# ucla-mobility/QuantV2X

Measured on AMD Instinct MI355X. Metric: frames/sec/node (N-agent int8 BEV fusion), higher is better.
Workload: dtype i8

## Files before the change

quantv2x_amd/csrc/codebook_encode_cand.hip:

```cpp
#include "common.h"

namespace qv2x {
namespace {

struct CandArgs {
    const int8_t* in; const int8_t* gpack; const double* bias; const int* tables;
    uint8_t* codes; unsigned* list; unsigned* counters;
    float tau[3][3];
    int n, h, w, hw, M, levels, kc, ke, zx, gbytes, tbytes;
    float delta;
};

constexpr int NPF = 8;
constexpr int LIMBS = 3;
template <int V> struct IC { static constexpr int value = V; };

__device__ __forceinline__ double shfl_xor_f64(double v, int m) {
    const long long b = __builtin_bit_cast(long long, v);
    const int lo = __shfl_xor((int)b, m), hi = __shfl_xor((int)(b >> 32), m);
    return __builtin_bit_cast(double, ((long long)hi << 32) | (unsigned)lo);
}

template <int CT, int SEGS, int PACK>
__global__ __launch_bounds__(256) __attribute__((amdgpu_waves_per_eu(1, 1))) void encode_candidates_kernel(const CandArgs a) {
    const int lane = threadIdx.x & 63, wave = __builtin_amdgcn_readfirstlane(threadIdx.x >> 6), j = lane & 31, hf = lane >> 5;
    const int m0 = ((int)blockIdx.x * 4 + wave) * (32 * CT);

    v4i xb[CT][8];
    int m[CT];
    float n0[CT], n1[CT];
#pragma unroll
    for (int ct = 0; ct < CT; ++ct) {
        m[ct] = m0 + 32 * ct + j;
        const int mc = m[ct] < a.M ? m[ct] : a.M - 1;
        const int img = mc / a.hw, rem = mc - img * a.hw, y = rem / a.w, x = rem - y * a.w;
        const int8_t* px = a.in + ((size_t)(img * (a.h + 2) + y + 1) * (a.w + 2) + x + 1) * 256 + 16 * hf;
#pragma unroll
        for (int s = 0; s < 8; ++s) xb[ct][s] = *(const v4i*)(px + 32 * s);
        unsigned s1 = 0, s2 = 0, sad = 0;
        const unsigned zx4 = (unsigned)a.zx * 0x01010101u;
#pragma unroll
        for (int s = 0; s < 8; ++s)
#pragma unroll
            for (int d = 0; d < 4; ++d) {
                const unsigned u = (unsigned)xb[ct][s][d] ^ 0x80808080u;
                s1 = __builtin_amdgcn_udot4(u, 0x01010101u, s1, false);
                s2 = __builtin_amdgcn_udot4(u, u, s2, false);
                sad = __builtin_amdgcn_sad_u8(u, zx4, sad);
            }
        s1 += __shfl_xor(s1, 32); s2 += __shfl_xor(s2, 32); sad += __shfl_xor(sad, 32);
        const int n2 = (int)s2 - 2 * a.zx * (int)s1 + 256 * a.zx * a.zx;
        n0[ct] = a.delta * sqrtf((float)n2);
        n1[ct] = (float)sad;
    }

    const __amdgpu_buffer_rsrc_t grs = __builtin_amdgcn_make_buffer_rsrc((void*)a.gpack, 0, a.gbytes, 0x00020000);
    int wo = 0;
    const int loff = lane * 16;
    auto gload = [&](int f) __attribute__((always_inline)) { return (v4i)__builtin_amdgcn_raw_buffer_load_b128(grs, loff, wo + f * 1024, 0); };
    v4i ring[NPF];
#pragma unroll
    for (int i = 0; i < NPF; ++i) ring[i] = gload(i);

    const __amdgpu_buffer_rsrc_t brs = __builtin_amdgcn_make_buffer_rsrc((void*)a.bias, 0, a.levels * a.ke * 8, 0x00020000);
    const __amdgpu_buffer_rsrc_t trs = __builtin_amdgcn_make_buffer_rsrc((void*)a.tables, 0, a.tbytes, 0x00020000);
    int o[2][SEGS][CT] = {};
    int first[CT];
#pragma unroll
    for (int ct = 0; ct < CT; ++ct) first[ct] = 3;
    const int ntile = a.kc >> 5;
    const int tsz = a.ke * a.ke;
    auto level = [&](auto lc) __attribute__((always_inline)) {
        constexpr int l = decltype(lc)::value;
        bool weak_l[CT];
#pragma unroll
        for (int ct = 0; ct < CT; ++ct) weak_l[ct] = false;
        auto segment = [&](auto sc) __attribute__((always_inline)) {
        constexpr int sg = decltype(sc)::value;
        double best[CT], second[CT];
#pragma unroll
        for (int ct = 0; ct < CT; ++ct) best[ct] = second[ct] = 1.0e300;
        v4i qb[2][2], qt[2][l > 0 ? l * SEGS : 1][CT];
        auto issue = [&](int T, int g, int slot) __attribute__((always_inline)) {
            const int col = sg * a.kc + 32 * T + 8 * g;
            const int kofs = l * a.ke + col;
            qb[slot][0] = (v4i)__builtin_amdgcn_raw_buffer_load_b128(brs, 32 * hf, kofs * 8, 0);
            qb[slot][1] = (v4i)__builtin_amdgcn_raw_buffer_load_b128(brs, 32 * hf + 16, kofs * 8, 0);
#pragma unroll
            for (int ct = 0; ct < CT; ++ct) {
#pragma unroll
                for (int jj = 0; jj < l; ++jj)
#pragma unroll
                    for (int sp = 0; sp < SEGS; ++sp)
                        qt[slot][jj * SEGS + sp][ct] = (v4i)__builtin_amdgcn_raw_buffer_load_b128(trs, o[jj][sp][ct], ((l * (l - 1) / 2 + jj) * tsz + col) * 4, 0);
            }
        };
#pragma unroll 1
        for (int T = 0; T < ntile; ++T) {
            v16i acc[LIMBS][CT];
#pragma unroll
            for (int lb = 0; lb < LIMBS; ++lb)
#pragma unroll
                for (int ct = 0; ct < CT; ++ct)
#pragma unroll
                    for (int r = 0; r < 16; ++r) acc[lb][ct][r] = 0;
#pragma unroll
            for (int f = 0; f < LIMBS * 8; ++f) {
                const v4i A = ring[f % NPF];
#pragma unroll
                for (int ct = 0; ct < CT; ++ct) acc[f >> 3][ct] = __builtin_amdgcn_mfma_i32_32x32x32_i8(A, xb[ct][f & 7], acc[f >> 3][ct], 0, 0, 0);
                ring[f % NPF] = gload(f + NPF);
                if (f == LIMBS * 8 - 6) issue(T, 0, 0);
                __builtin_amdgcn_sched_barrier(0);
            }
            wo += LIMBS * 8 * 1024;
#pragma unroll
            for (int g = 0; g < 4; ++g) {
                if (g < 3) issue(T, g + 1, (g + 1) & 1);
                __builtin_amdgcn_sched_barrier(0);
                const int sl = g & 1;
                double b[4];
                b[0] = __builtin_bit_cast(double, ((unsigned long long)(unsigned)qb[sl][0][1] << 32) | (unsigned)qb[sl][0][0]);
                b[1] = __builtin_bit_cast(double, ((unsigned long long)(unsigned)qb[sl][0][3] << 32) | (unsigned)qb[sl][0][2]);
                b[2] = __builtin_bit_cast(double, ((unsigned long long)(unsigned)qb[sl][1][1] << 32) | (unsigned)qb[sl][1][0]);
                b[3] = __builtin_bit_cast(double, ((unsigned long long)(unsigned)qb[sl][1][3] << 32) | (unsigned)qb[sl][1][2]);
#pragma unroll
                for (int ct = 0; ct < CT; ++ct) {
#pragma unroll
                    for (int e = 0; e < 4; ++e) {
                        const int r = 4 * g + e;
                        int lo = (acc[1][ct][r] << 8) + acc[0][ct][r];
#pragma unroll
                        for (int q = 0; q < l * SEGS; ++q) lo += qt[sl][q][ct][e];
                        double c = __builtin_fma((double)lo, (double)PACK, b[e]);
                        c = __builtin_fma((double)acc[2][ct][r], 65536.0 * PACK, c);
                        second[ct] = fmin(second[ct], fmax(best[ct], c));
                        best[ct] = fmin(best[ct], c);
                    }
                }
                __builtin_amdgcn_sched_barrier(0);
            }
        }
#pragma unroll
        for (int ct = 0; ct < CT; ++ct) {
            const double ob = shfl_xor_f64(best[ct], 32), os = shfl_xor_f64(second[ct], 32);
            const double nb = fmin(best[ct], ob), ns = fmin(fmax(best[ct], ob), fmin(second[ct], os));
            const int c = (int)((long long)nb & (PACK - 1));
            if (l < 2) o[l < 2 ? l : 0][sg][ct] = ((sg * a.kc + c) * a.ke + 4 * hf) * 4;
            const float t = ((a.tau[l][0] + a.tau[l][1] * n0[ct]) + (a.tau[l][2] * n0[ct]) * n0[ct]) + n1[ct];
            weak_l[ct] |= !(ns - nb > (double)PACK * (double)ceilf(t) + (double)(PACK - 1));
            if (hf == 0 && m[ct] < a.M) a.codes[(size_t)(l * SEGS + sg) * a.M + m[ct]] = (uint8_t)c;
        }
        };
        segment(IC<0>{});
        if constexpr (SEGS > 1) segment(IC<1>{});
#pragma unroll
        for (int ct = 0; ct < CT; ++ct)
            if (weak_l[ct] && first[ct] == 3) first[ct] = l;
    };
    level(IC<0>{});
    if (a.levels > 1) level(IC<1>{});
    if (a.levels > 2) level(IC<2>{});
    unsigned long long mask[3][CT];
    unsigned cnt[3] = {0, 0, 0};
#pragma unroll
    for (int c = 0; c < 3; ++c)
#pragma unroll
        for (int ct = 0; ct < CT; ++ct) {
            mask[c][ct] = __builtin_amdgcn_ballot_w64(first[ct] == c && hf == 0 && m[ct] < a.M);
            cnt[c] += (unsigned)__builtin_popcountll(mask[c][ct]);
        }
    __shared__ unsigned wcnt[4][3], wbase[3];
    if (lane == 0) { wcnt[wave][0] = cnt[0]; wcnt[wave][1] = cnt[1]; wcnt[wave][2] = cnt[2]; }
    __syncthreads();
    if (threadIdx.x < 3) {
        const unsigned tot = wcnt[0][threadIdx.x] + wcnt[1][threadIdx.x] + wcnt[2][threadIdx.x] + wcnt[3][threadIdx.x];
        wbase[threadIdx.x] = tot ? atomicAdd(a.counters + 1 + threadIdx.x, tot) : 0u;
        if (tot) atomicAdd(a.counters, tot);
    }
    __syncthreads();
    unsigned base[3];
#pragma unroll
    for (int c = 0; c < 3; ++c) {
        base[c] = wbase[c];
        for (int w2 = 0; w2 < wave; ++w2) base[c] += wcnt[w2][c];
    }
#pragma unroll
    for (int c = 0; c < 3; ++c) {
        unsigned at = __builtin_amdgcn_readfirstlane(base[c]);
#pragma unroll
        for (int ct = 0; ct < CT; ++ct) {
            if (first[ct] == c && hf == 0 && m[ct] < a.M)
                a.list[(size_t)c * a.M + at + (unsigned)__builtin_popcountll(mask[c][ct] & ((1ull << lane) - 1ull))] = (unsigned)m[ct];
            at += (unsigned)__builtin_popcountll(mask[c][ct]);
        }
    }
}

__global__ void zero_counters_kernel(unsigned* c) { if (threadIdx.x < 4) c[threadIdx.x] = 0; }

template <int CT, int SEGS, int PACK>
void launch(const CandArgs& a, hipStream_t st) {
    encode_candidates_kernel<CT, SEGS, PACK><<<(a.M + 128 * CT - 1) / (128 * CT), 256, 0, st>>>(a);
}

template <int PACK, int MAX_SEGS>
int candidates(const char* me, const qv2x_encode_desc* d, const int8_t* in, const int8_t* g_limbs, const double* bias_packed, const int32_t* tables,
               const float* tau, uint8_t* codes, uint32_t* list, uint32_t* counters, void* stream) {
    if (!d || !in || !g_limbs || !bias_packed || !tau || !codes || !list || !counters) return fail(QV2X_EINVAL, "%s: null pointer", me);
    if (d->n <= 0 || d->h <= 0 || d->w <= 0 || d->levels < 1 || d->levels > 3) return fail(QV2X_EINVAL, "%s: 1..3 levels", me);
    const int segs = d->segs ? d->segs : 1;
    if (segs < 1 || segs > MAX_SEGS) return fail(QV2X_EINVAL, "%s: seg_num 1 .. %d (got %d; the exact entry takes seg_num 1 | 2 | 4)", me, MAX_SEGS, d->segs);
    if (d->kc < 32 || d->kc > PACK || d->kc % 32 || (segs > 1 && d->kc % 64))
        return fail(QV2X_EINVAL, "%s: dict_size a multiple of 32 up to %d (of 64 with two segments; got %d x %d)", me, PACK, segs, d->kc);
    if (d->levels > 1 && !tables) return fail(QV2X_EINVAL, "%s: the residual levels need their tables", me);
    if (d->in_zx < 0 || d->in_zx > 255) return fail(QV2X_EINVAL, "%s: in_zx outside 0..255", me);
    if (((uintptr_t)in & 15) || ((uintptr_t)g_limbs & 15) || ((uintptr_t)tables & 15) || ((uintptr_t)bias_packed & 7))
        return fail(QV2X_EALIGN, "%s: 16-byte aligned maps, limbs and tables", me);
    CandArgs a;
    a.in = in; a.gpack = g_limbs; a.bias = bias_packed; a.tables = tables; a.codes = codes; a.list = list; a.counters = counters;
    for (int l = 0; l < 3; ++l)
        for (int i = 0; i < 3; ++i) a.tau[l][i] = l < d->levels ? tau[l * 3 + i] : 0.0f;
    a.n = d->n; a.h = d->h; a.w = d->w; a.hw = d->h * d->w; a.M = d->n * a.hw; a.levels = d->levels; a.kc = d->kc; a.ke = segs * d->kc; a.zx = d->in_zx;
    a.gbytes = d->levels * (a.ke / 32) * LIMBS * 8 * 1024;
    a.tbytes = (d->levels > 1 ? d->levels * (d->levels - 1) / 2 : 1) * a.ke * a.ke * 4;
    a.delta = d->in_delta;
    hipStream_t st = (hipStream_t)stream;
    zero_counters_kernel<<<1, 64, 0, st>>>(counters);
    int dev = 0, cus = 256, v = 0;
    if (hipGetDevice(&dev) == hipSuccess && hipDeviceGetAttribute(&v, hipDeviceAttributeMultiprocessorCount, dev) == hipSuccess && v > 0) cus = v;
    const bool large = a.M >= 4 * cus * 32 * (segs == 2 ? 3 : 4) * 2;
    if (segs == 1) large ? launch<4, 1, PACK>(a, st) : launch<2, 1, PACK>(a, st);
    else if constexpr (MAX_SEGS > 1) large ? launch<3, 2, PACK>(a, st) : launch<2, 2, PACK>(a, st);
    return hip_check(hipGetLastError(), me);
}

}
}

extern "C" int qv2x_codebook_encode_candidates_i8(const qv2x_encode_desc* d, const int8_t* in, const int8_t* g_limbs, const double* bias_packed,
                                                  const int32_t* tables, const float* tau, uint8_t* codes, uint32_t* list, uint32_t* counters,
                                                  void* stream) {
    return qv2x::candidates<128, 1>("qv2x_codebook_encode_candidates_i8", d, in, g_limbs, bias_packed, tables, tau, codes, list, counters, stream);
}

extern "C" int qv2x_codebook_encode_candidates_seg_i8(const qv2x_encode_desc* d, const int8_t* in, const int8_t* g_limbs, const double* bias_packed,
                                                      const int32_t* tables, const float* tau, uint8_t* codes, uint32_t* list, uint32_t* counters,
                                                      void* stream) {
    return qv2x::candidates<256, 2>("qv2x_codebook_encode_candidates_seg_i8", d, in, g_limbs, bias_packed, tables, tau, codes, list, counters, stream);
}
```

quantv2x_amd/csrc/codebook_encode_wave.hip:

```cpp
#include "codebook_encode.h"

namespace qv2x {

namespace {

constexpr int D = ENC_D;
constexpr int RS = 260;
constexpr int NPF = 4;

__device__ __forceinline__ v16f mfma(float a, float b, v16f c) { return __builtin_amdgcn_mfma_f32_32x32x2f32(a, b, c, 0, 0, 0); }


__device__ __forceinline__ void tile_to_lds(float* __restrict__ row, int h, int T, const v16f& acc) {
#pragma unroll
    for (int rq = 0; rq < 4; ++rq) {
        float* g = row + (4 * T + rq) * 8 + 2 * h;
        *(float2*)g = make_float2(acc[4 * rq], acc[4 * rq + 2]);
        *(float2*)(g + 4) = make_float2(acc[4 * rq + 1], acc[4 * rq + 3]);
    }
}

__device__ __forceinline__ void lds_to_operand(const float* __restrict__ row, int h, float (&m)[128]) {
#pragma unroll
    for (int g = 0; g < 32; ++g) {
        const v4f v = *(const v4f*)(row + g * 8 + 4 * h);
        m[4 * g] = v.x; m[4 * g + 1] = v.y; m[4 * g + 2] = v.z; m[4 * g + 3] = v.w;
    }
}

__device__ __forceinline__ void tile_vec(const float* __restrict__ p, int h, int T, v4f (&o)[4]) {
#pragma unroll
    for (int rq = 0; rq < 4; ++rq) o[rq] = *(const v4f*)(p + 32 * T + 8 * rq + 4 * h);
}

#ifdef QV2X_ENCW_FINE
__device__ long long g_encw_fine[4096][32];
#define WFINE(k) do { if (threadIdx.x == 0 && blockIdx.x < 4096) g_encw_fine[blockIdx.x][8 * l + (k)] = __builtin_readcyclecounter(); } while (0)
#define WFINE2(k) do { if (fine2 && threadIdx.x == 0 && blockIdx.x < 4096) g_encw_fine[blockIdx.x][24 + (k)] = __builtin_readcyclecounter(); } while (0)
#define WFINE2_ARM(v) fine2 = (v)
#else
#define WFINE(k) do { } while (0)
#define WFINE2(k) do { } while (0)
#define WFINE2_ARM(v) do { } while (0)
#endif

}

template <int V> struct IC { static constexpr int value = V; };

template <bool F32IN, int SEGS, bool LIST = false>
__global__ __attribute__((amdgpu_flat_work_group_size(64, 64), amdgpu_waves_per_eu(1, 1))) void codebook_encode_wave_kernel(const EncArgs a) {
    __shared__ __attribute__((aligned(16))) float smem[32 * RS];
    const int lane = threadIdx.x, j = lane & 31, h = lane >> 5;
    float* const row = smem + j * RS;
    ListPlan plan{};
    if (LIST) plan = list_plan(a);
#pragma unroll 1
    for (int round = 0; LIST ? round * (int)gridDim.x < plan.full : round == 0; ++round) {
    const int tile = LIST ? round * (int)gridDim.x + ((round & 1) ? (int)gridDim.x - 1 - (int)blockIdx.x : (int)blockIdx.x) : (int)blockIdx.x;
    if (LIST && tile >= plan.full) continue;
    int mrow;
    bool owned;
    int start = 0;
    if (LIST) {
        int cls, i0;
        list_tile(plan, tile, cls, i0);
        owned = i0 + j < plan.n[cls];
        mrow = (int)a.list[(size_t)cls * a.M + (owned ? i0 + j : plan.n[cls] - 1)];
        start = cls;
    } else {
        mrow = a.m_lo + tile * 32 + j;
        owned = mrow < a.m_hi;
    }

    float xq[128], z[128];
    {
        int m = mrow;
        m = m < a.M ? m : a.M - 1;
        const int img = m / (a.h * a.w), rem = m - img * (a.h * a.w);
        const int y = rem / a.w, x = rem - y * a.w;
        const size_t pixel = (size_t)(img * (a.h + 2) + y + 1) * (a.w + 2) + x + 1;
        if (F32IN) {
            const v4f* sf = (const v4f*)(a.in_f32 + pixel * D);
#pragma unroll
            for (int q = 0; q < 64; ++q) {
                const v4f v = sf[q];
                xq[2 * q] = h ? v.y : v.x;
                xq[2 * q + 1] = h ? v.w : v.z;
            }
        } else {
            const v4i* src = (const v4i*)(a.in + pixel * D);
            const float fax = (float)(a.ax - 128);
#pragma unroll
            for (int c = 0; c < 16; ++c) {
                const v4i raw = src[c];
#pragma unroll
                for (int d = 0; d < 4; ++d) {
                    const unsigned u = ((unsigned)raw[d] ^ 0x80808080u) >> (8 * h);
                    xq[8 * c + 2 * d] = ((float)(u & 0xffu) + fax) * a.dx;
                    xq[8 * c + 2 * d + 1] = ((float)((u >> 16) & 0xffu) + fax) * a.dx;
                }
            }
        }
    }

    for (int l = 0; l < a.levels; ++l) {
        const float* W = a.lvl[l];
        const float* stage_b = W + D * D;
        const float* qhead_b = stage_b + D + D * D;
        const float* lhead_b = qhead_b + D + D * D;
        const float* cb = lhead_b + D + (size_t)D * a.ke;
        const float* c2 = cb + (size_t)a.ke * D;
        const __amdgpu_buffer_rsrc_t wrs = __builtin_amdgcn_make_buffer_rsrc((void*)(W + level_floats_wg(a.ke)), 0, 0x7fffffff, 0x00020000);
        int wo = 0;
        const int loff = lane * 16;
        auto wload = [&](int grp) __attribute__((always_inline)) {
            return __builtin_bit_cast(v4f, __builtin_amdgcn_raw_buffer_load_b128(wrs, loff, wo + grp * 1024, 0));
        };
        const bool last = l + 1 == a.levels;
        const int npair = (a.ke + 63) >> 6;

        v4f bn[2][4];
        auto next_vec = [&](const float* p, int P) __attribute__((always_inline)) {
            tile_vec(p, h, 2 * P, bn[0]);
            tile_vec(p, h, 2 * P + 1, bn[1]);
        };
        auto next_c2 = [&](int P) __attribute__((always_inline)) {
            tile_vec(c2, h, 2 * P, bn[0]);
            if (64 * P + 32 < a.ke) tile_vec(c2, h, 2 * P + 1, bn[1]);
            else
#pragma unroll
                for (int i = 0; i < 4; ++i) bn[1][i] = v4f{INFINITY, INFINITY, INFINITY, INFINITY};
        };
        auto next_c2s = [&](int s0, int s1, int P) __attribute__((always_inline)) {
            tile_vec(c2 + s0 * a.kc, h, P, bn[0]);
            tile_vec(c2 + s1 * a.kc, h, P, bn[1]);
        };
        next_vec(stage_b, 0);
        __builtin_amdgcn_sched_barrier(0);
        v4f ring[2 * NPF];
#pragma unroll
        for (int i = 0; i < 2 * NPF; ++i) ring[i] = wload(i);
        __builtin_amdgcn_sched_barrier(0);

        v16f acc[2];
#ifdef QV2X_ENCW_FINE
        bool fine2 = false;
#endif
        auto tile2g = [&](const float (&m)[128], const bool biased, auto&& hook, auto ng_c, auto off0_c, auto off1_c) __attribute__((always_inline)) {
            constexpr int NG = decltype(ng_c)::value, OFF0 = decltype(off0_c)::value, OFF1 = decltype(off1_c)::value;
            WFINE2(0);
#pragma unroll
            for (int t = 0; t < 2; ++t)
#pragma unroll
                for (int r = 0; r < 16; ++r) acc[t][r] = biased ? bn[t][r >> 2][r & 3] : 0.0f;
            WFINE2(1);
#pragma unroll
            for (int g = 0; g < NG; ++g) {
                const v4f A0 = ring[(2 * g) % (2 * NPF)], A1 = ring[(2 * g + 1) % (2 * NPF)];
                acc[0] = mfma(A0.x, m[OFF0 + 4 * g], acc[0]);
                acc[1] = mfma(A1.x, m[OFF1 + 4 * g], acc[1]);
                __builtin_amdgcn_sched_barrier(0);
                acc[0] = mfma(A0.y, m[OFF0 + 4 * g + 1], acc[0]);
                acc[1] = mfma(A1.y, m[OFF1 + 4 * g + 1], acc[1]);
                __builtin_amdgcn_sched_barrier(0);
                acc[0] = mfma(A0.z, m[OFF0 + 4 * g + 2], acc[0]);
                acc[1] = mfma(A1.z, m[OFF1 + 4 * g + 2], acc[1]);
                __builtin_amdgcn_sched_barrier(0);
                acc[0] = mfma(A0.w, m[OFF0 + 4 * g + 3], acc[0]);
                acc[1] = mfma(A1.w, m[OFF1 + 4 * g + 3], acc[1]);
                if (g == NG - NPF - 1) hook();
                if (NG == 32 && g == 7) WFINE2(2);
                if (NG == 32 && g == 15) WFINE2(3);
                if (NG == 32 && g == 23) WFINE2(4);
#ifndef QV2X_ENCW_ABL_NOLOAD
                ring[(2 * g) % (2 * NPF)] = wload(2 * (g + NPF));
                ring[(2 * g + 1) % (2 * NPF)] = wload(2 * (g + NPF) + 1);
#endif
                __builtin_amdgcn_sched_barrier(0);
            }
#ifndef QV2X_ENCW_ABL_SAMEW
            wo += NG * 2048;
#endif
            WFINE2(5);
        };
        auto tile2 = [&](const float (&m)[128], const bool biased, auto&& hook) __attribute__((always_inline)) {
            tile2g(m, biased, hook, IC<32>{}, IC<0>{}, IC<0>{});
        };

        WFINE(0);
#pragma unroll 1
        for (int P = 0; P < 4; ++P) {
            WFINE2_ARM(l == 1 && P == 1);
            tile2(xq, true, [&]() __attribute__((always_inline)) { next_vec(P < 3 ? stage_b : qhead_b, P < 3 ? P + 1 : 0); });
            tile_to_lds(row, h, 2 * P, acc[0]);
            tile_to_lds(row, h, 2 * P + 1, acc[1]);
            WFINE2(6);
            WFINE2_ARM(false);
        }
        WFINE(1);
        lds_to_operand(row, h, z);
        WFINE(2);
        unsigned bcs = 0;
        if (LIST && l < start) {
            wo = SEGS == 1 ? (8 + npair) * 65536 : 8 * 65536 + (SEGS / 2) * (a.kc >> 5) * (32 / SEGS) * 2048;
            next_vec(lhead_b, 0);
#pragma unroll
            for (int i = 0; i < 2 * NPF; ++i) ring[i] = wload(i);
#pragma unroll
            for (int sg = 0; sg < SEGS; ++sg) bcs |= (unsigned)a.codes[((size_t)l * SEGS + sg) * a.M + mrow] << (8 * sg);
        } else {
#pragma unroll 1
        for (int P = 0; P < 4; ++P) {
            tile2(z, true, [&]() __attribute__((always_inline)) { if (P < 3) next_vec(qhead_b, P + 1); else if (SEGS == 1) next_c2(0); else next_c2s(0, 1, 0); });
            tile_to_lds(row, h, 2 * P, acc[0]);
            tile_to_lds(row, h, 2 * P + 1, acc[1]);
        }
        WFINE(3);
        lds_to_operand(row, h, xq);
        float x2s[4];
        {
            const float* qh = row + 128 * h;
            float p[2];
#pragma unroll
            for (int c = 0; c < 2; ++c) {
                float s = 0.0f;
#pragma unroll
                for (int g = 0; g < 8; ++g) {
                    const v4f e = *(const v4f*)(qh + (8 * c + g) * 8), o = *(const v4f*)(qh + (8 * c + g) * 8 + 4);
                    s = fmaf(e.x, e.x, s); s = fmaf(o.x, o.x, s); s = fmaf(e.y, e.y, s); s = fmaf(o.y, o.y, s);
                    s = fmaf(e.z, e.z, s); s = fmaf(o.z, o.z, s); s = fmaf(e.w, e.w, s); s = fmaf(o.w, o.w, s);
                }
                p[c] = s;
            }
            const float mine = p[0] + p[1];
            const float other = __shfl_xor(mine, 32);
            if (a.segs == 1) {
                x2s[0] = x2s[1] = x2s[2] = x2s[3] = mine + other;
            } else if (a.segs == 2) {
                x2s[0] = h ? other : mine; x2s[1] = h ? mine : other; x2s[2] = x2s[3] = 0.0f;
            } else {
                const float o0 = __shfl_xor(p[0], 32), o1 = __shfl_xor(p[1], 32);
                x2s[0] = h ? o0 : p[0]; x2s[1] = h ? o1 : p[1]; x2s[2] = h ? p[0] : o0; x2s[3] = h ? p[1] : o1;
            }
        }
        WFINE(4);
        if constexpr (SEGS == 1) {
        float best = INFINITY;
        int bc = 0;
        const int ppseg = npair / a.segs;
#pragma unroll 1
        for (int P = 0; P < npair; ++P) {
            const int seg = a.segs == 1 ? 0 : P / ppseg, cbase = seg * a.kc;
            const float x2 = seg == 0 ? x2s[0] : (seg == 1 ? x2s[1] : (seg == 2 ? x2s[2] : x2s[3]));
            v4f c2t[2][4];
#pragma unroll
            for (int t = 0; t < 2; ++t)
#pragma unroll
                for (int i = 0; i < 4; ++i) c2t[t][i] = bn[t][i];
            tile2(xq, false, [&]() __attribute__((always_inline)) { if (P + 1 < npair) next_c2(P + 1); else if (!last) next_vec(lhead_b, 0); });
#pragma unroll
            for (int t = 0; t < 2; ++t)
#pragma unroll
                for (int r = 0; r < 16; ++r) {
                    const float s = x2 + c2t[t][r >> 2][r & 3];
                    const float d = s - 2.0f * acc[t][r];
                    const int code = 64 * P + 32 * t + 8 * (r >> 2) + 4 * h + (r & 3) - cbase;
                    const bool lt = d < best;
                    best = lt ? d : best;
                    bc = lt ? code : bc;
                }
            if (a.segs == 1 ? P + 1 == npair : (P + 1) % ppseg == 0) {
                const float od = __shfl_xor(best, 32);
                const int oc = __shfl_xor(bc, 32);
                if (od < best || (od == best && oc < bc)) bc = oc;
                if (h == 0 && owned) a.codes[((size_t)l * a.segs + seg) * a.M + mrow] = (uint8_t)bc;
                bcs |= (unsigned)bc << (8 * seg);
                best = INFINITY; bc = 0;
            }
        }
        } else {
            const int ntile = a.kc >> 5;
            auto seg_pairs = [&](auto sa_c, auto sb_c, const bool more_after) __attribute__((always_inline)) {
                constexpr int SA = decltype(sa_c)::value, SB = decltype(sb_c)::value, NG = 32 / SEGS;
                float best[2] = {INFINITY, INFINITY};
                int bc[2] = {0, 0};
#pragma unroll 1
                for (int P = 0; P < ntile; ++P) {
                    v4f c2t[2][4];
#pragma unroll
                    for (int t = 0; t < 2; ++t)
#pragma unroll
                        for (int i = 0; i < 4; ++i) c2t[t][i] = bn[t][i];
                    tile2g(xq, false, [&]() __attribute__((always_inline)) {
                        if (P + 1 < ntile) next_c2s(SA, SB, P + 1);
                        else if (more_after) next_c2s(SA + 2, SB + 2, 0);
                        else if (!last) next_vec(lhead_b, 0);
                    }, IC<NG>{}, IC<4 * NG * SA>{}, IC<4 * NG * SB>{});
#pragma unroll
                    for (int t = 0; t < 2; ++t) {
                        const float x2 = x2s[t ? SB : SA];
#pragma unroll
                        for (int r = 0; r < 16; ++r) {
                            const float sv = x2 + c2t[t][r >> 2][r & 3];
                            const float d = sv - 2.0f * acc[t][r];
                            const int code = 32 * P + 8 * (r >> 2) + 4 * h + (r & 3);
                            const bool lt = d < best[t];
                            best[t] = lt ? d : best[t];
                            bc[t] = lt ? code : bc[t];
                        }
                    }
                }
#pragma unroll
                for (int t = 0; t < 2; ++t) {
                    const int seg = t ? SB : SA;
                    const float od = __shfl_xor(best[t], 32);
                    const int oc = __shfl_xor(bc[t], 32);
                    if (od < best[t] || (od == best[t] && oc < bc[t])) bc[t] = oc;
                    if (h == 0 && owned) a.codes[((size_t)l * SEGS + seg) * a.M + mrow] = (uint8_t)bc[t];
                    bcs |= (unsigned)bc[t] << (8 * seg);
                }
            };
            if constexpr (SEGS == 2) seg_pairs(IC<0>{}, IC<1>{}, false);
            else { seg_pairs(IC<0>{}, IC<1>{}, true); seg_pairs(IC<2>{}, IC<3>{}, false); }
        }
        }
        WFINE(5);
        if (last) break;
#pragma unroll 1
        for (int P = 0; P < 4; ++P) {
            const int seg = (P * a.segs) >> 2;
            const float* cw = cb + (size_t)(seg * a.kc + (int)((bcs >> (8 * seg)) & 0xffu)) * D;
            v4f cv[2][4];
            tile_vec(cw, h, 2 * P, cv[0]);
            tile_vec(cw, h, 2 * P + 1, cv[1]);
            __builtin_amdgcn_sched_barrier(0);
            tile2(z, true, [&]() __attribute__((always_inline)) { if (P < 3) next_vec(lhead_b, P + 1); });
#pragma unroll
            for (int t = 0; t < 2; ++t) {
#pragma unroll
                for (int r = 0; r < 16; ++r) acc[t][r] = acc[t][r] - cv[t][r >> 2][r & 3];
                tile_to_lds(row, h, 2 * P + t, acc[t]);
            }
        }
        WFINE(6);
        lds_to_operand(row, h, xq);
        WFINE(7);
    }
    }
}

int encode_wave_launch(const EncArgs& a, hipStream_t st) {
    const unsigned grid = (unsigned)((a.m_hi - a.m_lo + 31) / 32);
    if (a.segs == 2) {
        if (a.in_f32) codebook_encode_wave_kernel<true, 2><<<grid, 64, 0, st>>>(a);
        else codebook_encode_wave_kernel<false, 2><<<grid, 64, 0, st>>>(a);
    } else if (a.segs == 4) {
        if (a.in_f32) codebook_encode_wave_kernel<true, 4><<<grid, 64, 0, st>>>(a);
        else codebook_encode_wave_kernel<false, 4><<<grid, 64, 0, st>>>(a);
    } else if (a.in_f32) codebook_encode_wave_kernel<true, 1><<<grid, 64, 0, st>>>(a);
    else codebook_encode_wave_kernel<false, 1><<<grid, 64, 0, st>>>(a);
    return hip_check(hipGetLastError(), "qv2x_codebook_encode_f32 (wave form) launch");
}


int encode_wave_list_launch(const EncArgs& a, int waves, hipStream_t st) {
    if ((a.segs != 1 && a.segs != 2) || a.in_f32) return fail(QV2X_EINVAL, "qv2x_codebook_encode_listed_f32: seg_num 1 | 2, i8 rows");
    if (a.segs == 2) codebook_encode_wave_kernel<false, 2, true><<<(unsigned)waves, 64, 0, st>>>(a);
    else codebook_encode_wave_kernel<false, 1, true><<<(unsigned)waves, 64, 0, st>>>(a);
    return hip_check(hipGetLastError(), "qv2x_codebook_encode_listed_f32 launch");
}

}

#ifdef QV2X_ENCW_FINE
extern "C" __attribute__((visibility("default"))) int qv2x_debug_encw_fine(long long* host, int n) {
    return hipMemcpyFromSymbol(host, HIP_SYMBOL(qv2x::g_encw_fine), (size_t)n * 32 * sizeof(long long)) == hipSuccess ? 0 : -1;
}
#endif
```

quantv2x_amd/encode_two_stage.py:

```python
from typing import Dict

import numpy as np

U = 2.0 ** -24
LIMBS = 3
G_MAX_INT = 2 ** 23 - 2 ** 15 - 2 ** 7 - 1


def _sn(m):
    return float(np.linalg.norm(m, 2)) if m.size else 0.0


def _kappa(w, block=8):
    k = w.shape[1]
    return float(sum(min(block, k - i0) * _sn(w[:, :min(k, i0 + block)]) for i0 in range(0, k, block)))


class _Aff:

    def __init__(self, p=0.0, r=0.0):
        self.p, self.r = float(p), float(r)

    def __add__(self, o):
        return _Aff(self.p + o.p, self.r + o.r)
# ... 66 lines not shown

CANDIDATE_ENTRY = {128: "qv2x_codebook_encode_candidates_i8", 256: "qv2x_codebook_encode_candidates_seg_i8"}


def candidate_tables(state: Dict[str, np.ndarray], levels: int, in_delta: float, in_zx: int, segs: int = 1) -> Dict[str, np.ndarray]:
    from .engine import collapse_encoder_f64
    G, gb, tabs = collapse_encoder_f64(state, levels)
    ke = G.shape[0] // levels
    kc = ke // segs
    if any(state[f"codebook/{l}/codebook"].shape[0] != ke for l in range(levels)):
        raise ValueError("two-stage encode: every level needs the same dict_size")
    if segs == 1:
        if kc % 32 or kc > 256 or levels > 3:
            raise ValueError("two-stage encode: dict_size 32 | 64 | 96 | 128 | ... | 256, up to three levels")
    elif segs != 2 or kc * segs != ke or kc % 64 or kc > 256 or levels > 3:
        raise ValueError("two-stage encode: seg_num 1 | 2, dict_size a multiple of 64 up to 256 with two segments, up to three levels")
    n_t = segs * max(levels - 1, 0)
    tlim = 2.0 ** 29 / max(2, n_t)
    blim = 2.0 ** 44 if pack_factor(segs, kc) == 128 else 2.0 ** 43
    gs = float(in_delta) * G
    tmax = max([float(np.abs(t).max()) for t in tabs.values()] + [0.0])
    h = max(float(np.abs(gs).max()) / G_MAX_INT, tmax / (tlim - 2.0), float(np.abs(gb).max()) / (blim - 2.0 ** 32))
    gi = np.rint(gs / h).astype(np.int64)
    limbs, rest = [], gi.copy()
    for _ in range(LIMBS):
        d = ((rest + 128) % 256) - 128
        limbs.append(d.astype(np.int8))
        rest = (rest - d) // 256
    if rest.any():
        raise ValueError("two-stage encode: G on the grid does not fit the candidate stage's int8 limbs")
    bias = np.rint(gb / h).astype(np.int64) + (128 - int(in_zx)) * gi.sum(1)
    tables = np.stack([np.rint(tabs[(l, j)] / h) for l in range(levels) for j in range(l)]) if levels > 1 else np.zeros((1, ke, ke))
    if np.abs(tables).max() >= tlim or np.abs(bias).max() >= blim:
        raise ValueError("two-stage encode: table / bias entries leave the fixed-point range of the candidate stage")
    lane = np.arange(64)
    score = (np.arange(levels * ke // 32)[:, None, None, None] * 32 + (lane & 31)[None, None, :, None])
    chan = (32 * np.arange(8)[None, :, None, None] + 16 * (lane >> 5)[None, None, :, None] + np.arange(16)[None, None, None, :])
    packed = np.stack([lb[score, chan] for lb in limbs], axis=1)
    packed = packed.reshape(levels, ke // 32, LIMBS, 8, 64, 16)
    ea, eb, ec, report = encode_error_bound(state, levels, in_delta, segs)
    fp = 1.0 + 1e-4
    tau = np.zeros((levels, 3))
    for l in range(levels):
        own = 1.0 + segs * l + 2.0
        tau[l] = [(ea[l] / h + own) * fp, eb[l] / h * fp, ec[l] / h * fp]
    return {"gpack": np.ascontiguousarray(packed, dtype=np.int8), "bias": np.ascontiguousarray(bias, dtype=np.int64),
            "tables": np.ascontiguousarray(tables, dtype=np.int32), "tau": np.ascontiguousarray(tau, dtype=np.float32), "h": h,
            "g_int": gi, "bound": (ea, eb, ec), "report": report, "segs": segs, "kc": kc, "pack": pack_factor(segs, kc)}


def candidate_emulate(codes_u8: np.ndarray, tabs: Dict[str, np.ndarray], in_delta: float, in_zx: int):
    gi, bias, tables, tau, h = tabs["g_int"], tabs["bias"], tabs["tables"], tabs["tau"], tabs["h"]
    levels = tau.shape[0]
    segs = int(tabs.get("segs", 1))
    ke = gi.shape[0] // levels
    kc = ke // segs
    P = float(tabs.get("pack", 128))
    b = codes_u8.astype(np.float64) - 128.0
    s = b @ gi.astype(np.float64).T + bias.astype(np.float64)[None]
    n = codes_u8.astype(np.int64) - int(in_zx)
    n1, n2 = np.abs(n).sum(1), (n * n).sum(1)
    n0 = (np.float32(in_delta) * np.sqrt(n2.astype(np.float32))).astype(np.float32)
    out = np.zeros((levels * segs, codes_u8.shape[0]), np.uint8)
    flags = np.zeros((levels * segs, codes_u8.shape[0]), bool)
    gaps = np.zeros((levels * segs, codes_u8.shape[0]))
    for l in range(levels):
        sc = s[:, l * ke:(l + 1) * ke].copy()
        for j in range(l):
            for sp in range(segs):
                sc += tables[l * (l - 1) // 2 + j][sp * kc + out[j * segs + sp].astype(np.int64)].astype(np.float64)
        t = (((tau[l, 0] + tau[l, 1] * n0) + (tau[l, 2] * n0) * n0) + n1.astype(np.float32)).astype(np.float32)
        assert t.dtype == np.float32 and n0.dtype == np.float32
        t = t.astype(np.float64)
        for sg in range(segs):
            v = sc[:, sg * kc:(sg + 1) * kc]
            order = np.argsort(v, axis=1, kind="stable")
            best, second = np.take_along_axis(v, order[:, :1], 1)[:, 0], np.take_along_axis(v, order[:, 1:2], 1)[:, 0]
            p = l * segs + sg
            out[p] = order[:, 0]
            k2 = order[:, 1]
            flags[p] = (P * second + k2) - (P * best + out[p]) <= P * np.ceil(t) + (P - 1.0)
            gaps[p] = (second - best) * h
    return out, flags.any(0), flags, gaps
```

quantv2x_amd/engine.py:

```python
from __future__ import annotations

import ctypes as C
from typing import Dict, List, Optional

import numpy as np
import torch
import torch.nn as nn

from . import lib as L
from .ptq_state import export_ptq_state, load_ptq_state

_HEADS = ("cls_head", "reg_head", "dir_head")


def _dev(a: np.ndarray, dev) -> torch.Tensor:
    return torch.from_numpy(np.ascontiguousarray(a)).to(dev).contiguous()


def _pack_k4(w: np.ndarray) -> np.ndarray:
    j, k = w.shape
    assert k % 4 == 0
    return np.ascontiguousarray(w.T.reshape(k // 4, 4, j).transpose(0, 2, 1), dtype=np.float32)


# ... 624 lines not shown
        b["canvas_clean"] = True

    def encode_codes(self, n_agents: int, out: Optional[torch.Tensor] = None):
        b = self._workspace(n_agents)
        codes = b["codes"] if out is None else out
        if codes.dtype != torch.uint8 or not codes.is_contiguous() or codes.numel() != self.levels * n_agents * self.fh * self.fw:
            raise ValueError("encode_codes: out must be a contiguous uint8 tensor [levels, n_agents, H*W]")
        d = L.EncodeDesc()
        d.n, d.h, d.w, d.levels, d.kc, d.segs = n_agents, self.fh, self.fw, self.enc_levels, self.kc, self.segs
        d.in_zx, d.in_delta = int(self.shrink1.out_q[1]), float(self.shrink1.out_q[0])
        two_stage = self.encode_mode == "two_stage" and self.encode_form == "auto"
        if two_stage and self._two_stage is None:
            self._refuse_during_capture("encode_mode 'two_stage'")
            self._build_two_stage()
            two_stage = self.encode_mode == "two_stage"
        if self.encode_mode == "collapsed":
            if self.segs != 1 or self.kc > 128:
                raise NotImplementedError("encode_mode 'collapsed': seg_num 1 and dict_size <= 128 (the exact encode takes the rest)")
            if self._collapsed is None:
                self._refuse_during_capture("encode_mode 'collapsed'")
                self._collapsed = tuple(_dev(t, self.dev) for t in collapse_encoder(self.state, self.enc_levels, d.in_delta, d.in_zx))
            gp, bias, tab = self._collapsed
            L.check(self.lib.qv2x_codebook_encode_collapsed_f32(C.byref(d), L.ptr(b["s1"]), L.ptr(gp), L.ptr(bias), L.ptr(tab), L.ptr(codes),
                                                                L.current_stream()), "qv2x_codebook_encode_collapsed_f32")
            return codes
        if two_stage:
            return self._encode_two_stage(d, b, codes)
        if self.encode_mode not in ("exact", "two_stage"):
            raise ValueError(f"encode_mode {self.encode_mode!r}: 'exact' (every cell through the reference's op order), 'two_stage' (the same "
                             "indices: exact integer candidates, the chain only where the bound cannot decide) or 'collapsed' (opt-in, approximate)")
        if self.encode_form == "wave":
            L.check(self.lib.qv2x_codebook_encode_wave_f32(C.byref(d), L.ptr(b["s1"]), None, self.level_ptrs, L.ptr(codes),
                                                           L.current_stream()), "qv2x_codebook_encode_wave_f32")
            return codes
        L.check(self.lib.qv2x_codebook_encode_f32(C.byref(d), L.ptr(b["s1"]), self.level_ptrs, L.ptr(codes),
                                                  L.current_stream()), "qv2x_codebook_encode_f32")
        return codes

    def two_stage_supported(self) -> bool:
        if not self.has_codebook or self.enc_levels > 3 or self.kc > 256:
            return False
        return bool(self.kc % 32 == 0 if self.segs == 1 else self.segs == 2 and self.kc % 64 == 0)

    def _refuse_during_capture(self, what: str):
        if torch.cuda.is_current_stream_capturing():
            raise L.Qv2xError(f"{what}: its operands are built on the host and uploaded -- not inside a HIP-graph capture; encode once "
                              "in this mode before capturing")

    def _build_two_stage(self):
        if not self.two_stage_supported():
            raise NotImplementedError("encode_mode 'two_stage': seg_num 1 | 2, dict_size <= 256, up to three levels (encode_mode 'exact' takes the rest)")
        from .encode_two_stage import candidate_tables
        try:
            t = candidate_tables(self.state, self.enc_levels, float(self.shrink1.out_q[0]), int(self.shrink1.out_q[1]), self.segs)
            k = np.arange(t["bias"].shape[0], dtype=np.int64) % self.kc
            pf = int(t["pack"])
            packed = (pf * t["bias"] + k).astype(np.float64)
            if not np.array_equal(packed.astype(np.int64), pf * t["bias"] + k):
                raise ValueError("two-stage encode: packed scores not exact in float64")
            self._two_stage = (_dev(t["gpack"], self.dev), _dev(packed, self.dev), _dev(t["tables"], self.dev),
                               (C.c_float * (3 * self.enc_levels))(*[float(v) for v in t["tau"].reshape(-1)]), t)
        except Exception as e:
            self.encode_mode, self.two_stage_refused = "exact", str(e) or type(e).__name__

    def candidate_entry(self) -> str:
        from .encode_two_stage import CANDIDATE_ENTRY, pack_factor
        return CANDIDATE_ENTRY[pack_factor(self.segs, self.kc)]

    def _encode_two_stage(self, d, b, codes):
        gp, bias, tab, tau, _ = self._two_stage
        name = self.candidate_entry()
        L.check(getattr(self.lib, name)(C.byref(d), L.ptr(b["s1"]), L.ptr(gp), L.ptr(bias), L.ptr(tab), tau, L.ptr(codes),
                                        L.ptr(b["enc_list"]), L.ptr(b["enc_counters"]), L.current_stream()), name)
        L.check(self.lib.qv2x_codebook_encode_listed_f32(C.byref(d), L.ptr(b["s1"]), self.level_ptrs, L.ptr(b["enc_list"]), L.ptr(b["enc_counters"]),
                                                         L.ptr(codes), L.current_stream()), "qv2x_codebook_encode_listed_f32")
        return codes

    def encode_refine_stats(self, n_agents: int) -> dict:
        if not (self.encode_mode == "two_stage" and self.encode_form == "auto") or "enc_counters" not in self._bufs.get(n_agents, {}):
            raise L.Qv2xError(f"encode_refine_stats({n_agents}): no two-stage encode of {n_agents} frames here (encode_mode "
                              f"{self.encode_mode!r}, encode_form {self.encode_form!r}, workspaces {sorted(self._bufs)})")
        c = self._bufs[n_agents]["enc_counters"].cpu().numpy().astype(np.int64)
        cells = n_agents * self.fh * self.fw
        return {"cells": cells, "refined": int(c[0]), "refined_fraction": float(c[0]) / cells, "first_flagged_at_level": [int(v) for v in c[1:1 + self.enc_levels]]}

    def wire_shape(self):
        self._workspace(1)
        return self.levels, self.fh * self.fw

    def encode_into(self, inputs: dict, frames: int, codes_out: torch.Tensor):
        self.pillars_to_canvas(inputs, frames, resident=True)
        try:
            self.run_plan(frames)
            self.clear_pillars(inputs, frames)
        except BaseException:
            self._restore_canvas(frames)
            raise
        return self.encode_codes(frames, out=codes_out)

    def pairwise_from_poses(self, gathered: torch.Tensor, world: int, agent_stride: int, pose_offset: int, max_cav: int, out: torch.Tensor):
        L.check(self.lib.qv2x_pairwise_from_poses_f64(L.ptr(gathered), world, agent_stride, pose_offset, max_cav, L.ptr(out),
                                                      L.current_stream()), "qv2x_pairwise_from_poses_f64")

    def pairwise_frames_from_poses(self, gathered: torch.Tensor, world: int, agent_stride: int, pose_offset: int, frames: int, frame_stride: int,
                                   max_cav: int, out: torch.Tensor):
        L.check(self.lib.qv2x_pairwise_from_poses_batch_f64(L.ptr(gathered), world, agent_stride, pose_offset, frames, frame_stride, max_cav,
                                                            L.ptr(out), L.current_stream()), "qv2x_pairwise_from_poses_batch_f64")

    def fuse_frames_and_heads(self, gathered: torch.Tensor, agent_stride: int, level_stride: int, frame_stride: int, pairwise: torch.Tensor,
                              n_agents: int, ego: int, own_codes: Optional[torch.Tensor], frames: int) -> dict:
        lens = [n_agents] * frames
        form = self._post_form(lens, None, own_codes is not None and frame_stride == self.fh * self.fw)
        return self._post(form, L.ptr(gathered), agent_stride, level_stride, None, pairwise, [f * frame_stride for f in range(frames)], lens, ego,
                          own_codes, frames)

    def band_shape(self):
        self._workspace(1)
        return self.heads.cout, self.fh, self.fw

    def head_wire_supported(self, wire: str) -> bool:
        if wire not in L.WIRES:
            raise ValueError(f"wire: one of {sorted(L.WIRES)}, got {wire!r}")
        return wire == "f32" or bool((self.heads.da_np > 0).all())

    def fuse_frames_and_heads_band(self, gathered: torch.Tensor, agent_stride: int, level_stride: int, frame_stride: int, pairwise: torch.Tensor,
                                   n_agents: int, ego: int, frames: int, y0: int, y1: int, out_slab: torch.Tensor, wire: str = "f32"):
        if not self.head_wire_supported(wire):
            raise L.Qv2xError("band wire 'u8': a head without an output quantizer has no codes to send")
        hd, n_cells, esz = self.heads, (y1 - y0) * self.fw, (1 if wire == "u8" else 4)
        if not 0 <= y0 <= y1 <= self.fh:
            raise ValueError(f"band rows [{y0}, {y1}) outside the map's {self.fh} rows")
        if out_slab.dtype != torch.uint8 or out_slab.numel() < frames * hd.cout * n_cells * esz:
            raise ValueError("out_slab: u8, at least frames * cout * band cells * element size bytes")
        if n_cells == 0:
            return
        one_launch = self.band_one_launch
        if one_launch is None:
            one_launch = frames * n_cells // 32 >= self.fuse_heads_min_tiles and n_agents <= self._one_launch_agents()
        rows = None
        if not one_launch:
            key = (frames, n_cells)
            if self._band_rows is None or self._band_rows[0] != key:
                self._band_rows = (key, torch.empty((frames, n_cells, 256), dtype=torch.float32, device=self.dev))
            rows = self._band_rows[1]
        lut = L.ptr(self.lut) if self.has_codebook else None
        lb = L.ptr(self.lut_bias) if self.has_codebook else None
        base, st = out_slab.data_ptr(), L.current_stream()
        for s0 in range(0, frames, 64):
            s1 = min(frames, s0 + 64)
            d = self._fuse_desc(agent_stride, level_stride, pairwise[s0], n_agents, ego)
            offs = (C.c_int64 * (s1 - s0))(*[f * frame_stride for f in range(s0, s1)])
            cnts = (C.c_int32 * (s1 - s0))(*([n_agents] * (s1 - s0)))
            out = C.c_void_p(base + s0 * hd.cout * n_cells * esz)
            if one_launch:
                L.check(self.lib.qv2x_fuse_heads_band(C.byref(d), s1 - s0, offs, cnts, L.ptr(gathered), lut, lb, None, L.ptr(pairwise[s0]),
                                                      y0 * self.fw, n_cells, hd.cout, hd.cout_pad, L.ptr(hd.w), L.ptr(hd.bias), L.ptr(hd.da),
                                                      L.ptr(hd.za), L.WIRES[wire], L.ptr(hd.da_np), out, None, st), "qv2x_fuse_heads_band")
            else:
                L.check(self.lib.qv2x_fuse_att_band_f32(C.byref(d), s1 - s0, offs, cnts, L.ptr(gathered), lut, lb, None, L.ptr(pairwise[s0]),
                                                        y0 * self.fw, n_cells, L.ptr(rows[s0]), st), "qv2x_fuse_att_band_f32")
                L.check(self.lib.qv2x_heads_band(L.ptr(rows[s0]), s1 - s0, n_cells, hd.cout, hd.cout_pad, L.ptr(hd.w), L.ptr(hd.bias),
                                                 L.ptr(hd.da), L.ptr(hd.za), L.WIRES[wire], L.ptr(hd.da_np), out, st), "qv2x_heads_band")

    def assemble_bands(self, gathered_slabs: torch.Tensor, world: int, frames: int, wire: str, out: torch.Tensor):
        hd = self.heads
        L.check(self.lib.qv2x_assemble_bands(L.ptr(gathered_slabs), world, gathered_slabs.shape[1], frames, hd.cout, self.fh, self.fw, L.WIRES[wire],
                                             L.ptr(hd.da), L.ptr(hd.za), L.ptr(out), L.current_stream()), "qv2x_assemble_bands")
# ... 292 lines not shown
```

Measured before the change: 6943.

## Record per-level undecided masks and let refine stop early on confirmed cells

The candidate kernel now records a bitmask of every level where a cell was undecided, not only the first one, and stores it as a byte at the tail of the list buffer. The refine kernel uses this mask in two ways. Cells that are undecided again at later levels are compacted into dense windows. Cells undecided only at their first level stop after that level once the refined code matches the candidate code wave-wide. This is meant to skip the exact refinement of later levels when the cheap candidates are already correct, at the cost of extra tile scheduling, LDS compaction and byte flags packed into the unused end of the list buffer.

```diff
diff --git a/quantv2x_amd/csrc/codebook_encode_cand.hip b/quantv2x_amd/csrc/codebook_encode_cand.hip
--- a/quantv2x_amd/csrc/codebook_encode_cand.hip
+++ b/quantv2x_amd/csrc/codebook_encode_cand.hip
@@ -65,9 +65,9 @@
     const __amdgpu_buffer_rsrc_t brs = __builtin_amdgcn_make_buffer_rsrc((void*)a.bias, 0, a.levels * a.ke * 8, 0x00020000);
     const __amdgpu_buffer_rsrc_t trs = __builtin_amdgcn_make_buffer_rsrc((void*)a.tables, 0, a.tbytes, 0x00020000);
     int o[2][SEGS][CT] = {};
-    int first[CT];
-#pragma unroll
-    for (int ct = 0; ct < CT; ++ct) first[ct] = 3;
+    int und[CT];
+#pragma unroll
+    for (int ct = 0; ct < CT; ++ct) und[ct] = 0;
     const int ntile = a.kc >> 5;
     const int tsz = a.ke * a.ke;
     auto level = [&](auto lc) __attribute__((always_inline)) {
@@ -156,11 +156,14 @@
         if constexpr (SEGS > 1) segment(IC<1>{});
 #pragma unroll
         for (int ct = 0; ct < CT; ++ct)
-            if (weak_l[ct] && first[ct] == 3) first[ct] = l;
+            if (weak_l[ct]) und[ct] |= 1 << l;
     };
     level(IC<0>{});
     if (a.levels > 1) level(IC<1>{});
     if (a.levels > 2) level(IC<2>{});
+    int first[CT];
+#pragma unroll
+    for (int ct = 0; ct < CT; ++ct) first[ct] = und[ct] ? __builtin_ctz((unsigned)und[ct]) : 3;
     unsigned long long mask[3][CT];
     unsigned cnt[3] = {0, 0, 0};
 #pragma unroll
@@ -190,8 +193,11 @@
         unsigned at = __builtin_amdgcn_readfirstlane(base[c]);
 #pragma unroll
         for (int ct = 0; ct < CT; ++ct) {
-            if (first[ct] == c && hf == 0 && m[ct] < a.M)
-                a.list[(size_t)c * a.M + at + (unsigned)__builtin_popcountll(mask[c][ct] & ((1ull << lane) - 1ull))] = (unsigned)m[ct];
+            if (first[ct] == c && hf == 0 && m[ct] < a.M) {
+                const unsigned pos = at + (unsigned)__builtin_popcountll(mask[c][ct] & ((1ull << lane) - 1ull));
+                a.list[(size_t)c * a.M + pos] = (unsigned)m[ct];
+                if (c + 1 < a.levels) ((uint8_t*)(a.list + (size_t)(c + 2) * a.M))[-1 - (ptrdiff_t)pos] = (uint8_t)und[ct];
+            }
             at += (unsigned)__builtin_popcountll(mask[c][ct]);
         }
     }
diff --git a/quantv2x_amd/csrc/codebook_encode_wave.hip b/quantv2x_amd/csrc/codebook_encode_wave.hip
--- a/quantv2x_amd/csrc/codebook_encode_wave.hip
+++ b/quantv2x_amd/csrc/codebook_encode_wave.hip
@@ -54,20 +54,57 @@
     const int lane = threadIdx.x, j = lane & 31, h = lane >> 5;
     float* const row = smem + j * RS;
     ListPlan plan{};
-    if (LIST) plan = list_plan(a);
-#pragma unroll 1
-    for (int round = 0; LIST ? round * (int)gridDim.x < plan.full : round == 0; ++round) {
-    const int tile = LIST ? round * (int)gridDim.x + ((round & 1) ? (int)gridDim.x - 1 - (int)blockIdx.x : (int)blockIdx.x) : (int)blockIdx.x;
-    if (LIST && tile >= plan.full) continue;
+    __shared__ int dslot[LIST ? 256 : 1];
+    int nwin[2] = {0, 0}, nvirt = 0;
+    if (LIST) {
+        plan = list_plan(a);
+        for (int c = 0; c < 2; ++c) nwin[c] = c + 1 < a.levels ? (plan.n[c] + 255) >> 8 : 0;
+        nvirt = nwin[0] + nwin[1] + plan.full;
+    }
+    const int undmask = LIST ? (1 << a.levels) - 1 : 0;
+#pragma unroll 1
+    for (int round = 0; LIST ? round * (int)gridDim.x < nvirt : round == 0; ++round) {
+    const int tile = LIST ? round * (int)gridDim.x + (((round + 1) & 2) ? (int)gridDim.x - 1 - (int)blockIdx.x : (int)blockIdx.x) : (int)blockIdx.x;
+    if (LIST && tile >= nvirt) continue;
+    int npass = 1, wcls = 0, wcount = 0;
+    const bool window = LIST && tile < nwin[0] + nwin[1];
+    if (window) {
+        wcls = tile < nwin[0] ? 0 : 1;
+        const int i0 = (tile - (wcls ? nwin[0] : 0)) << 8;
+        const uint8_t* ftop = (const uint8_t*)(a.list + (size_t)(wcls + 2) * a.M) - 1;
+        __syncthreads();
+        for (int r = 0; r < 4; ++r) {
+            const int i = i0 + 64 * r + lane;
+            const bool dirty = i < plan.n[wcls] && (((unsigned)ftop[-(ptrdiff_t)(i < plan.n[wcls] ? i : 0)] & undmask) >> (wcls + 1)) != 0;
+            const unsigned long long mk = __builtin_amdgcn_ballot_w64(dirty);
+            if (dirty) dslot[wcount + __builtin_popcountll(mk & ((1ull << lane) - 1ull))] = i;
+            wcount += __builtin_popcountll(mk);
+        }
+        __syncthreads();
+        npass = (wcount + 31) >> 5;
+    }
+#pragma unroll 1
+    for (int pass = 0; pass < npass; ++pass) {
     int mrow;
     bool owned;
     int start = 0;
+    bool vote = false;
     if (LIST) {
-        int cls, i0;
-        list_tile(plan, tile, cls, i0);
-        owned = i0 + j < plan.n[cls];
-        mrow = (int)a.list[(size_t)cls * a.M + (owned ? i0 + j : plan.n[cls] - 1)];
-        start = cls;
+        if (window) {
+            owned = 32 * pass + j < wcount;
+            mrow = (int)a.list[(size_t)wcls * a.M + dslot[owned ? 32 * pass + j : wcount - 1]];
+            start = wcls;
+        } else {
+            int cls, i0;
+            list_tile(plan, plan.full - 1 - (tile - nwin[0] - nwin[1]), cls, i0);
+            owned = i0 + j < plan.n[cls];
+            const int i = owned ? i0 + j : plan.n[cls] - 1;
+            mrow = (int)a.list[(size_t)cls * a.M + i];
+            start = cls;
+            vote = cls + 1 < a.levels;
+            if (vote && (((unsigned)((const uint8_t*)(a.list + (size_t)(cls + 2) * a.M))[-1 - (ptrdiff_t)i] & undmask) >> (cls + 1)) != 0)
+                owned = false;
+        }
     } else {
         mrow = a.m_lo + tile * 32 + j;
         owned = mrow < a.m_hi;
@@ -202,6 +239,11 @@
         lds_to_operand(row, h, z);
         WFINE(2);
         unsigned bcs = 0;
+        unsigned cand = 0;
+        const bool check = LIST && vote && l == start;
+        if (check)
+#pragma unroll
+            for (int sg = 0; sg < SEGS; ++sg) cand |= (unsigned)a.codes[((size_t)l * SEGS + sg) * a.M + mrow] << (8 * sg);
         if (LIST && l < start) {
             wo = SEGS == 1 ? (8 + npair) * 65536 : 8 * 65536 + (SEGS / 2) * (a.kc >> 5) * (32 / SEGS) * 2048;
             next_vec(lhead_b, 0);
@@ -327,6 +369,7 @@
         }
         WFINE(5);
         if (last) break;
+        if (check && __builtin_amdgcn_ballot_w64(owned && bcs != cand) == 0) break;
 #pragma unroll 1
         for (int P = 0; P < 4; ++P) {
             const int seg = (P * a.segs) >> 2;
@@ -346,6 +389,7 @@
         WFINE(6);
         lds_to_operand(row, h, xq);
         WFINE(7);
+    }
     }
     }
 }
diff --git a/quantv2x_amd/encode_two_stage.py b/quantv2x_amd/encode_two_stage.py
--- a/quantv2x_amd/encode_two_stage.py
+++ b/quantv2x_amd/encode_two_stage.py
@@ -172,3 +172,32 @@
             flags[p] = (P * second + k2) - (P * best + out[p]) <= P * np.ceil(t) + (P - 1.0)
             gaps[p] = (second - best) * h
     return out, flags.any(0), flags, gaps
+
+
+def list_flags(lst: np.ndarray, m_cells: int, c: int, n: int) -> np.ndarray:
+    b = np.ascontiguousarray(lst).view(np.uint8)
+    top = 4 * m_cells * (c + 2) - 1
+    return b[top - n + 1:top + 1][::-1].copy()
+
+
+def set_list_flags(lst: np.ndarray, m_cells: int, c: int, flags: np.ndarray) -> None:
+    b = lst.view(np.uint8)
+    top = 4 * m_cells * (c + 2) - 1
+    b[top - len(flags) + 1:top + 1] = np.asarray(flags, np.uint8)[::-1]
+
+
+def refine_emulate(cand: np.ndarray, flags: np.ndarray, chain: np.ndarray, segs: int = 1) -> np.ndarray:
+    planes, rows = cand.shape
+    levels = planes // segs
+    und = np.stack([flags[l * segs:(l + 1) * segs].any(0) for l in range(levels)])
+    out = cand.copy()
+    listed = und.any(0)
+    first = np.where(listed, und.argmax(0), levels)
+    for c in range(levels):
+        mine = listed & (first == c)
+        later = und[c + 1:].any(0) if c + 1 < levels else np.zeros(rows, bool)
+        confirmed = (chain[c * segs:(c + 1) * segs] == cand[c * segs:(c + 1) * segs]).all(0)
+        full = mine & (later | ~confirmed)
+        out[c * segs:(c + 1) * segs, mine] = chain[c * segs:(c + 1) * segs][:, mine]
+        out[(c + 1) * segs:, full] = chain[(c + 1) * segs:][:, full]
+    return out
diff --git a/quantv2x_amd/engine.py b/quantv2x_amd/engine.py
--- a/quantv2x_amd/engine.py
+++ b/quantv2x_amd/engine.py
@@ -730,7 +730,18 @@
                               f"{self.encode_mode!r}, encode_form {self.encode_form!r}, workspaces {sorted(self._bufs)})")
         c = self._bufs[n_agents]["enc_counters"].cpu().numpy().astype(np.int64)
         cells = n_agents * self.fh * self.fw
-        return {"cells": cells, "refined": int(c[0]), "refined_fraction": float(c[0]) / cells, "first_flagged_at_level": [int(v) for v in c[1:1 + self.enc_levels]]}
+        from .encode_two_stage import list_flags
+        lst = self._bufs[n_agents]["enc_list"].cpu().numpy()
+        hist = [[0] * self.enc_levels for _ in range(self.enc_levels)]
+        for lv in range(self.enc_levels):
+            if lv + 1 == self.enc_levels:
+                hist[lv][lv] = int(c[1 + lv])
+                continue
+            f = list_flags(lst, cells, lv, int(c[1 + lv])) & ((1 << self.enc_levels) - 1)
+            for last in range(lv, self.enc_levels):
+                hist[lv][last] = int(((f >> (last + 1)) == 0).sum() - sum(hist[lv][lv:last]))
+        return {"cells": cells, "refined": int(c[0]), "refined_fraction": float(c[0]) / cells, "first_flagged_at_level": [int(v) for v in c[1:1 + self.enc_levels]],
+                "first_last_undecided": hist}
 
     def wire_shape(self):
         self._workspace(1)
```

Result: slower. 6816 (-1.8%).
